# pain7576/ddpg-trucktrailer

Measured on AMD Instinct MI355X. Metric: env-steps/s, higher is better.
Workload: dtype f64

## Files before the change

ddpg-trucktrailer_amd/csrc/ttenv.hip:

```cpp
#include <hip/hip_runtime.h>
#include <hip/hip_ext.h>

#include <cmath>
#include <cstdarg>
#include <cstdio>
#include <cstdlib>
#include <cstring>
#include <new>
#include <type_traits>
#include <vector>

#include "ttenv.h"
#include "tthost.h"
#include "ttphilox.h"

namespace {

#include "ttenv_math.h"
#include "ttenv_state.h"
#include "ttenv_step.h"
#include "ttenv_pose.h"
#include "ttenv_log.h"
#include "ttenv_hold.h"

#ifdef TT_STAMPS
#include "ttstamps.h"
__device__ unsigned long long g_stepblk[1024][2];
__device__ TTLog g_log_step;
#endif
#define TT_STEP_HEAD()                                                                                                                  \
    if (cursor) {                       \
        obs += (size_t)cursor[1] * n * OBS;                                                                                             \
        reward += (size_t)cursor[0] * n;                                                                                                \
        done += (size_t)cursor[0] * n;                                                                                                  \
    }                                                                                                                                   \
    const int block_first = blockIdx.x * BLOCK;                                                                                         \
    const int i = block_first + threadIdx.x;                                                                                            \
    const bool valid = i < n;                                                                                                           \
    const int nv = min(BLOCK, n - block_first);                                                                                         \
    float of[OBS];                                                                                                                      \
                                                                                                                                        \
    if (b.counter && i == 0) *b.counter += 1
#define TT_STEP_LOADS()                                                                                                                 \
    Env e;                                                                                                                              \
    load_env<PER_ENV>(P, b, i, e);                                                                                                      \
    float a = 0.f;                                                                                                                      \
    if (!RANDOM_POLICY) a = action[i]
#define TT_STEP_ACT()                                                                                                                   \
    if (RANDOM_POLICY) {                                                                                                                \
        a = random_action(policy_seed, (uint32_t)i, pk_steps(e.pk), b.episodes[i]);                                                     \
        if (action_out) action_out[i] = a;                                                                                              \
    }
#define TT_STEP_OUT()                                                                                                                   \
    if (P.nt) {                                                                                                                         \
        __builtin_nontemporal_store((float)o.total, reward + i);                                                                        \
        __builtin_nontemporal_store((uint8_t)(o.done ? 1 : 0), done + i);                                                               \
    } else {                                                                                                                            \
        reward[i] = (float)o.total;                                                                                                     \
        done[i] = o.done ? 1 : 0;                                                                                                       \
    }                                                                                                                                   \
    if (INFO) write_info(info, (size_t)n, i, e, o)
#define TT_STEP_RESET()                                                                                                                 \
    if (AUTO_RESET && o.done) {                                                                                                         \
        const uint32_t ep = b.episodes[i] + 1u;                                                                                         \
        b.episodes[i] = ep;                                                                                                             \
        double sx, sy, syaw;                                                                                                            \
        random_pose(P, seed, (uint32_t)i, ep, sx, sy, syaw);                                                                            \
        const Goal g0{P.gx, P.gy, P.sg, P.cg};                                                                                          \
        place_env(P, b, i, e, sx, sy, syaw, g0, P.gyaw, e.L2, of);                                                                      \
    }                                                                                                                                   \
    store_env(b, i, e)
#define TT_STEP_RETURN()                                                                                                                \
    ret += o.total;                                                                                                                     \
    lg.acc[i] = o.done ? 0.0 : ret;                               \
    const uint32_t len = pk_steps(e.pk)
#define TT_STEP_LAUNCH_COUNT()                                                                                                          \
    if (threadIdx.x == 0) {                                                                                                             \
        const unsigned long long launch = __hip_atomic_load(lg.hdr + LG_LAUNCHES, __ATOMIC_RELAXED, __HIP_MEMORY_SCOPE_AGENT);          \
        const unsigned long long t = atomic_add_agent(lg.hdr + LG_TICKET, 1ull);                                                        \
        if (t == gridDim.x - 1u) {                               \
            __hip_atomic_store(lg.hdr + LG_TICKET, 0ull, __ATOMIC_RELAXED, __HIP_MEMORY_SCOPE_AGENT);                                   \
            __hip_atomic_store(lg.hdr + LG_LAUNCHES, launch + 1ull, __ATOMIC_RELAXED, __HIP_MEMORY_SCOPE_AGENT);                        \
        }                                                                                                                               \
    }

template <bool PER_ENV, bool INFO, bool AUTO_RESET, bool RANDOM_POLICY>
__global__ __launch_bounds__(BLOCK) void k_step(const KParams P, const int n, const Bufs b,
                                                const float *__restrict__ action, float *__restrict__ action_out,
                                                float *__restrict__ obs, float *__restrict__ reward,
                                                uint8_t *__restrict__ done, const Info info, const uint64_t seed,
                                                const uint64_t policy_seed, const int *__restrict__ cursor) {
    __shared__ __attribute__((aligned(16))) float tile[BLOCK * OBS];
#ifdef TT_STAMPS
    if (threadIdx.x == 0 && blockIdx.x < 1024) g_stepblk[blockIdx.x][0] = wall_clock64();
#endif
    TT_STEP_HEAD();
    if (valid) {
        TT_STEP_LOADS();
        __builtin_amdgcn_sched_barrier(0);
        TT_STEP_ACT();
        StepOut o;
#ifdef TT_DBG_STEP_MEM_ONLY
        o = StepOut{};
        o.total = e.psi1 + a; o.done = false;
        e.psi1 += 1e-9; e.psi2 += e.x1 * 1e-12; e.d3 = e.d2; e.d2 = e.d1; e.d1 = e.prev; e.cum += e.closest * 1e-12;
#pragma unroll
        for (int j = 0; j < OBS; ++j) of[j] = (float)(e.x2 + j);
#else
        step_env(P, e, a, of, o);
#endif
        TT_STEP_OUT();
        TT_STEP_RESET();
    }
    store_obs_tile(tile, of, valid, obs, block_first, nv, P.nt != 0);
#ifdef TT_STAMPS
    asm volatile("s_waitcnt vmcnt(0)" ::: "memory");
    __syncthreads();
    if (threadIdx.x == 0 && blockIdx.x < 1024) {
        g_stepblk[blockIdx.x][1] = wall_clock64();
        tt_log_add(g_log_step, g_stepblk[blockIdx.x][0], g_stepblk[blockIdx.x][1]);
    }
#endif
}

template <bool PER_ENV, bool INFO, bool AUTO_RESET, bool RANDOM_POLICY>
__global__ __launch_bounds__(BLOCK) void k_step_log(const KParams P, const int n, const Bufs b,
                                                    const float *__restrict__ action, float *__restrict__ action_out,
                                                    float *__restrict__ obs, float *__restrict__ reward,
                                                    uint8_t *__restrict__ done, const Info info, const uint64_t seed,
                                                    const uint64_t policy_seed, const int *__restrict__ cursor,
                                                    const EpLog lg) {
    __shared__ __attribute__((aligned(16))) float tile[BLOCK * OBS];
    TT_STEP_HEAD();
    if (valid) {
        TT_STEP_LOADS();
        double ret = lg.acc[i];
        __builtin_amdgcn_sched_barrier(0);
        TT_STEP_ACT();
        StepOut o;
        step_env(P, e, a, of, o);
        TT_STEP_OUT();
        TT_STEP_RETURN();
        TT_STEP_RESET();
        log_append(lg, i, o.done, o.flags, o.final_bonus > 0.0, len, ret);
    }
    store_obs_tile(tile, of, valid, obs, block_first, nv, P.nt != 0);
    TT_STEP_LAUNCH_COUNT();
}

template <bool PER_ENV, bool INFO, bool AUTO_RESET, bool RANDOM_POLICY>
__global__ __launch_bounds__(BLOCK) void k_step_tally(const KParams P, const int n, const Bufs b,
                                                      const float *__restrict__ action, float *__restrict__ action_out,
                                                      float *__restrict__ obs, float *__restrict__ reward,
                                                      uint8_t *__restrict__ done, const Info info, const uint64_t seed,
                                                      const uint64_t policy_seed, const int *__restrict__ cursor,
                                                      const EpLog lg) {
    __shared__ __attribute__((aligned(16))) float tile[BLOCK * OBS];
    TT_STEP_HEAD();
    if (valid) {
        TT_STEP_LOADS();
        double ret = lg.acc[i];
        __builtin_amdgcn_sched_barrier(0);
        TT_STEP_ACT();
        StepOut o;
        step_env(P, e, a, of, o);
        TT_STEP_OUT();
        TT_STEP_RETURN();
        double s0 = 0.0, s1 = 0.0, s2 = 0.0;
        if (o.done) {
            const double *cold = b.cold + i;
            const size_t S = (size_t)P.npad;
            s0 = cold[C_SX * S]; s1 = cold[C_SY * S]; s2 = cold[C_SYAW * S];
        }
        TT_STEP_RESET();
        tally_append(P, lg, i, o, len, ret, s0, s1, s2);
    }
    store_obs_tile(tile, of, valid, obs, block_first, nv, P.nt != 0);
    TT_STEP_LAUNCH_COUNT();
}

template <bool PER_ENV>
__global__ __launch_bounds__(BLOCK) void k_rollout(const KParams P, const int n, const Bufs b, const int k_steps,
                                                   float *__restrict__ obs, float *__restrict__ reward_sum,
                                                   int32_t *__restrict__ episodes_done, const uint64_t seed,
                                                   const uint64_t policy_seed) {
    __shared__ __attribute__((aligned(16))) float tile[BLOCK * OBS];
    const int block_first = blockIdx.x * BLOCK;
    const int i = block_first + threadIdx.x;
    const bool valid = i < n;
    float of[OBS];
    if (valid) {
        Env e;
        load_env<PER_ENV>(P, b, i, e);
        uint32_t ep = b.episodes[i];
        double rsum = 0.0;
        int ndone = 0;
        for (int t = 0; t < k_steps; ++t) {
            const float a = random_action(policy_seed, (uint32_t)i, pk_steps(e.pk), ep);
            StepOut o;
            step_env(P, e, a, of, o);
            rsum += o.total;
            if (o.done) {
                ep += 1u;
                ndone += 1;
                double sx, sy, syaw;
                random_pose(P, seed, (uint32_t)i, ep, sx, sy, syaw);
                const Goal g0{P.gx, P.gy, P.sg, P.cg};
                place_env(P, b, i, e, sx, sy, syaw, g0, P.gyaw, e.L2, of);
            }
        }
// ... 60 lines not shown
    va_end(ap);
    if (e) std::memcpy(e->err, g_err, tthost::ERR_BYTES);
    return code;
}

#define TT_HANDLE(env)                                                                       \
    do {                                                                                     \
        if (!(env)) return fail(nullptr, TT_EINVAL, "%s: NULL handle", __func__);            \
    } while (0)
#define TT_ENTER(env)                                                                        \
    do {                                                                                     \
        TT_HANDLE(env);                                                                      \
        TT_HIP(env, hipSetDevice(env->device));                                              \
    } while (0)

#define TT_HIP(e, call)                                                                      \
    do {                                                                                     \
        hipError_t err_ = (call);                                                            \
        if (err_ != hipSuccess) return fail((e), TT_EHIP, "%s: %s", #call, hipGetErrorString(err_)); \
    } while (0)

#define TT_LAUNCH(env, ...)                                                                  \
    do {                                                                                     \
        __VA_ARGS__;                                                                         \
        TT_HIP(env, hipGetLastError());                                                      \
    } while (0)
#define TT_RUN(env, ...)                                                                     \
    do {                                                                                     \
        TT_HIP(env, hipSetDevice(env->device));                                              \
        TT_LAUNCH(env, __VA_ARGS__);                                                         \
        return TT_OK;                                                                        \
    } while (0)

inline int nt_stores_for(int npad) {
    static const long long thr = [] {
        const char *e = std::getenv("TT_NT_ENVS");
        return e ? std::atoll(e) : 2097152ll;
    }();
    return thr > 0 && npad >= thr ? 1 : 0;
}

KParams make_kparams(const tt_params &p, int npad) {
    KParams k{};
    k.v = p.v1x;
    k.v_over_L1 = p.v1x / p.L1;
    k.ho = p.hitch_offset;
    k.h = p.dt;
    k.L2 = p.L2;
    k.gx = p.goal[0]; k.gy = p.goal[1]; k.gyaw = p.goal[2];
    k.sg = std::sin(p.goal[2]); k.cg = std::cos(p.goal[2]);
    k.minx = p.map_min_x; k.maxx = p.map_max_x; k.miny = p.map_min_y; k.maxy = p.map_max_y;
    const double w = p.map_max_x - p.map_min_x, hgt = p.map_max_y - p.map_min_y;
    k.cx = (p.map_max_x + p.map_min_x) / 2; k.cy = (p.map_max_y + p.map_min_y) / 2;
    k.inv_hx = 1.0 / (w / 2); k.inv_hy = 1.0 / (hgt / 2);
    k.inv_M = 1.0 / std::sqrt(w * w + hgt * hgt);
    k.max_steer = p.max_steer;
    k.pos_thr = p.position_threshold; k.ori_thr = p.orientation_threshold;
    k.step_length = p.step_length;
    k.inv_step_length = 1.0 / p.step_length;
    for (int i = 0; i < 3; ++i) { k.rlo[i] = p.reset_lo[i]; k.rhi[i] = p.reset_hi[i]; }
    k.extra_steps = p.extra_steps; k.fixed_max = p.fixed_max_steps;
    k.term_mask = p.term_mask;
    k.npad = npad;
    k.stateless = p.stateless_reward;
    k.pool_m = 0;
    k.pool = nullptr;
    k.nt = nt_stores_for(npad);
    return k;
}

inline int grid_for(int n) { return (n + BLOCK - 1) / BLOCK; }

// ... 5 lines not shown

template <bool PER_ENV, bool INFO, bool RANDOM_POLICY>
void launch_step(tt_env *e, bool auto_reset, const float *action, float *action_out, float *obs, float *reward,
                 uint8_t *done, const Info &info, uint64_t policy_seed, hipStream_t s, const int *cursor = nullptr) {
    const dim3 g(grid_for(e->n)), b(BLOCK);
    hipEvent_t t0 = nullptr, t1 = nullptr;
    if (e->profiling && e->ev_used < e->ev_start.size()) {
        t0 = e->ev_start[e->ev_used];
        t1 = e->ev_stop[e->ev_used];
        e->ev_used += 1;
    }
    const auto launch = [&](auto kernel, const auto &...log) {
        hipExtLaunchKernelGGL(kernel, g, b, 0, s, t0, t1, 0, e->kp, e->n, e->b, action, action_out, obs, reward, done, info, e->seed,
                              policy_seed, cursor, log...);
    };
    if (e->task_dev && auto_reset) {
        const TaskDev *tk = e->task_dev;
        if (e->log_bytes) launch(k_step_task_log<INFO, RANDOM_POLICY>, e->log, tk);
        else launch(k_step_task<INFO, RANDOM_POLICY>, tk);
    } else if (e->rnd_dev && auto_reset) {
        const RndDev *rnd = e->rnd_dev;
        if (e->log_bytes) launch(k_step_rnd_log<INFO, RANDOM_POLICY>, e->log, rnd);
        else launch(k_step_rnd<INFO, RANDOM_POLICY>, rnd);
    } else if (e->cur_dev && auto_reset) {
        const CurDev *cur = e->cur_dev;
        if (e->log_bytes) launch(k_step_cur_log<PER_ENV, INFO, RANDOM_POLICY>, e->log, cur);
        else launch(k_step_cur<PER_ENV, INFO, RANDOM_POLICY>, cur);
    } else if (e->log_flags & TT_LOG_DETAIL) {
        if (auto_reset) launch(k_step_tally<PER_ENV, INFO, true, RANDOM_POLICY>, e->log);
        else launch(k_step_tally<PER_ENV, INFO, false, RANDOM_POLICY>, e->log);
    } else if (e->log_bytes) {
        if (auto_reset) launch(k_step_log<PER_ENV, INFO, true, RANDOM_POLICY>, e->log);
        else launch(k_step_log<PER_ENV, INFO, false, RANDOM_POLICY>, e->log);
    } else if (auto_reset)
        launch(k_step<PER_ENV, INFO, true, RANDOM_POLICY>);
    else
        launch(k_step<PER_ENV, INFO, false, RANDOM_POLICY>);
}

template <bool RANDOM_POLICY>
int step_common(tt_env *env, const float *action, float *action_out, float *obs, float *reward, uint8_t *done,
                const tt_info *info, int auto_reset, uint64_t policy_seed, hipStream_t stream, const int *cursor = nullptr) {
    Info ki{nullptr, nullptr, nullptr};
    bool want_info = false;
    if (info) {
        ki.comp = info->comp; ki.violation = info->violation; ki.flags = info->flags;
        want_info = ki.comp || ki.violation || ki.flags;
    }
    const auto launch = [&](auto per_env, auto with_info) {
        launch_step<decltype(per_env)::value, decltype(with_info)::value, RANDOM_POLICY>(env, auto_reset != 0, action, action_out, obs,
                                                                                         reward, done, ki, policy_seed, stream, cursor);
    };
    by_per_env(env, [&](auto per_env) {
        if (want_info) launch(per_env, std::true_type{});
        else launch(per_env, std::false_type{});
    });
    hipError_t err = hipGetLastError();
    if (err != hipSuccess) return fail(env, TT_EHIP, "tt_env_step launch: %s", hipGetErrorString(err));
    return TT_OK;
}

constexpr long long kLogMaxCapacity = 1ll << 28;
inline int log_acc_rows(uint32_t flags) { return (flags & TT_LOG_DETAIL) ? 1 + TT_LOG_NCOMP : 1; }
size_t log_acc_offset(long long cap, uint32_t flags) {
    return log_records_bytes((unsigned long long)cap) + ((flags & TT_LOG_DETAIL) ? tally_records_bytes((unsigned long long)cap) : 0);
}
// ... 1003 lines not shown
```

ddpg-trucktrailer_amd/csrc/ttenv_curriculum.h:

```cpp
#pragma once

struct CurDev {
    uint32_t *cell;
    uint32_t *cum;
    uint32_t *attempts, *successes;
    int C, nx, ny, nyaw;
    uint32_t *q;
    double *p;
    unsigned long long *seen;
    int mode, reserved_;
    double alpha, uniform;
    double lo[3], width[3];
    unsigned long long seed;
};

__device__ __forceinline__ void curriculum_pose(const CurDev *cur, uint64_t seed, uint32_t env, uint32_t episode, double &sx,
                                                double &sy, double &syaw) {
#pragma clang fp contract(off)
    uint32_t r[4];
    philox4x32(env, episode, 0u, 0x7452u, (uint32_t)seed, (uint32_t)(seed >> 32), r);
    const uint32_t *cum = cur->cum;
    const int C = cur->C;
    const uint32_t t = (uint32_t)(((unsigned long long)r[3] * (unsigned long long)cum[C - 1]) >> 32);
    uint32_t lo = 0u;
// ... 29 lines not shown
        ncell = (uint32_t)cur->C;                                                                                                       \
    }                                                                                                                                   \
    if (cl < ncell) __hip_atomic_fetch_add(cur->attempts + cl, 1u, __ATOMIC_RELAXED, __HIP_MEMORY_SCOPE_AGENT);                         \
    if (cl < ncell && o.final_bonus > 0.0) __hip_atomic_fetch_add(cur->successes + cl, 1u, __ATOMIC_RELAXED, __HIP_MEMORY_SCOPE_AGENT); \
    if (o.done) {                                                                                                                       \
        const uint32_t ep = *ep_ptr + 1u;                                                                                               \
        *ep_ptr = ep;                                                                                                                   \
        double sx, sy, syaw;                                                                                                            \
        curriculum_pose(cur, cur->seed, (uint32_t)i, ep, sx, sy, syaw);                                                                 \
        const Goal g0{P.gx, P.gy, P.sg, P.cg};                                                                                          \
        place_env(P, b, i, e, sx, sy, syaw, g0, P.gyaw, e.L2, of);                                                                      \
    }                                                                                                                                   \
    store_env(b, i, e)

template <bool PER_ENV, bool INFO, bool RANDOM_POLICY>
__global__ __launch_bounds__(BLOCK) void k_step_cur(const KParams P, const int n, const Bufs b,
                                                    const float *__restrict__ action, float *__restrict__ action_out,
                                                    float *__restrict__ obs, float *__restrict__ reward,
                                                    uint8_t *__restrict__ done, const Info info, const uint64_t seed,
                                                    const uint64_t policy_seed, const int *__restrict__ cursor,
                                                    const CurDev *cur_arg) {
    __shared__ __attribute__((aligned(16))) float tile[BLOCK * OBS];
    TT_STEP_HEAD();
    TT_STEP_CUR();
    if (valid) {
        TT_STEP_LOADS();
        __builtin_amdgcn_sched_barrier(0);
        TT_STEP_ACT();
        StepOut o;
        step_env(P, e, a, of, o);
        TT_STEP_OUT();
        TT_STEP_RESET_CURRICULUM();
    }
    store_obs_tile(tile, of, valid, obs, block_first, nv, P.nt != 0);
}

template <bool PER_ENV, bool INFO, bool RANDOM_POLICY>
__global__ __launch_bounds__(BLOCK) void k_step_cur_log(const KParams P, const int n, const Bufs b,
                                                        const float *__restrict__ action, float *__restrict__ action_out,
                                                        float *__restrict__ obs, float *__restrict__ reward,
                                                        uint8_t *__restrict__ done, const Info info, const uint64_t seed,
                                                        const uint64_t policy_seed, const int *__restrict__ cursor,
                                                        const EpLog lg, const CurDev *cur_arg) {
    __shared__ __attribute__((aligned(16))) float tile[BLOCK * OBS];
    TT_STEP_HEAD();
    TT_STEP_CUR();
    if (valid) {
        TT_STEP_LOADS();
        double ret = lg.acc[i];
        __builtin_amdgcn_sched_barrier(0);
        TT_STEP_ACT();
        StepOut o;
        step_env(P, e, a, of, o);
        TT_STEP_OUT();
        TT_STEP_RETURN();
        TT_STEP_RESET_CURRICULUM();
        log_append(lg, i, o.done, o.flags, o.final_bonus > 0.0, len, ret);
    }
    store_obs_tile(tile, of, valid, obs, block_first, nv, P.nt != 0);
    TT_STEP_LAUNCH_COUNT();
}

__global__ __launch_bounds__(BLOCK) void k_reset_curriculum(const KParams P, const int n, const Bufs b, const uint8_t *mask,
                                                            float *obs, const uint64_t seed, const CurDev *cur) {
    reset_lane(P, n, b, mask, obs, [&](uint32_t env, uint32_t episode, double &sx, double &sy, double &syaw) {
        curriculum_pose(cur, seed, env, episode, sx, sy, syaw);
    });
}

__global__ void k_curriculum_seed(CurDev *cur, const uint64_t seed) { cur->seed = seed; }

__global__ __launch_bounds__(BLOCK) void k_curriculum_unset(const int n, const int k, const int32_t *idx, uint32_t *cell) {
    const int j = blockIdx.x * BLOCK + threadIdx.x;
    int i;
    if (!lane_of_entry(idx, k, n, j, i)) return;
    cell[i] = TT_CURRICULUM_NO_CELL;
}

__global__ __launch_bounds__(BLOCK) void k_curriculum_update(const CurDev *cur) {
#pragma clang fp contract(off)
    __shared__ uint32_t part[BLOCK];
    const int C = cur->C, tid = threadIdx.x;
    const int per = (C + BLOCK - 1) / BLOCK;
    const int first = min(C, tid * per), last = min(C, first + per);
    const double alpha = cur->alpha, u = cur->uniform;
    const bool hard = cur->mode == TT_CURRICULUM_HARD;
    uint32_t sum = 0u;
    for (int c = first; c < last; ++c) {
        double p = cur->p[c];
        const uint32_t na = cur->attempts[c];
        if (na > 0u) {
            const uint32_t s = cur->successes[c];
// ... 28 lines not shown
```

ddpg-trucktrailer_amd/csrc/ttenv_hold.h:

```cpp
#pragma once

struct HoldCols {
    double *ret, *end;
    int32_t *len;
    uint8_t *live, *flags, *success;
};
__host__ __device__ inline size_t hold_block_bytes(int npad) { return (4 * sizeof(double) + sizeof(int32_t) + 3) * (size_t)npad; }
__host__ __device__ inline HoldCols hold_cols(void *block, int npad) {
    const size_t S = (size_t)npad;
    HoldCols c;
    c.ret = static_cast<double *>(block);
    c.end = c.ret + S;
    c.len = reinterpret_cast<int32_t *>(c.end + 3 * S);
    c.live = reinterpret_cast<uint8_t *>(c.len + S);
    c.flags = c.live + S;
    c.success = c.flags + S;
    return c;
}

__device__ inline void load_obs_tile(float *tile, const float *obs, int block_first, int nv) {
    const int tid = threadIdx.x;
    const float *src = obs + (size_t)block_first * OBS;
    const int total = nv * OBS;
    if ((reinterpret_cast<uintptr_t>(src) & 15u) == 0) {
// ... 10 lines not shown

template <bool PER_ENV>
__global__ __launch_bounds__(BLOCK) void k_step_hold(const KParams P, const int n, const Bufs b, const float *__restrict__ mu,
                                                     const float action_scale, float *__restrict__ obs, void *const hold) {
    __shared__ __attribute__((aligned(16))) float tile[BLOCK * OBS];
    const int block_first = blockIdx.x * BLOCK;
    const int i = block_first + threadIdx.x;
    const int nv = min(BLOCK, n - block_first);
    const HoldCols h = hold_cols(hold, P.npad);
    const bool live = i < n && h.live[i] != 0;
    const int nlive = __syncthreads_count(live ? 1 : 0);
    if (nlive == 0) return;
    if (nlive < nv) load_obs_tile(tile, obs, block_first, nv);
    float of[OBS];
    if (live) {
        Env e;
        load_env<PER_ENV>(P, b, i, e);
        float a = mu[i];
        __builtin_amdgcn_sched_barrier(0);
        a = a * action_scale;
        StepOut o;
        step_env(P, e, a, of, o);
        h.ret[i] += o.total;
        store_env(b, i, e);
        if (o.done) {
            const size_t S = (size_t)P.npad;
            h.len[i] = (int32_t)pk_steps(e.pk);
            h.flags[i] = (uint8_t)o.flags;
            h.success[i] = o.final_bonus > 0.0 ? 1 : 0;
            h.end[i] = e.x2; h.end[S + i] = e.y2; h.end[2 * S + i] = e.psi2;
            h.live[i] = 0;
        }
    }
    store_obs_tile(tile, of, live, obs, block_first, nv, P.nt != 0);
}

__global__ __launch_bounds__(BLOCK) void k_hold_begin(const int n, const int npad, void *const hold) {
    const int i = blockIdx.x * BLOCK + threadIdx.x;
    if (i >= npad) return;
    const HoldCols h = hold_cols(hold, npad);
    const size_t S = (size_t)npad;
    h.live[i] = i < n ? 1 : 0;
    h.ret[i] = 0.0;
    h.len[i] = 0;
    h.flags[i] = 0;
    h.success[i] = 0;
    h.end[i] = 0.0; h.end[S + i] = 0.0; h.end[2 * S + i] = 0.0;
}

__global__ __launch_bounds__(BLOCK) void k_hold_live(const int npad, const void *const hold, long long *out) {
    __shared__ long long part[BLOCK];
    const uint32_t *w = reinterpret_cast<const uint32_t *>(hold_cols(const_cast<void *>(hold), npad).live);
    long long s = 0;
    for (int q = threadIdx.x; q < (npad >> 2); q += BLOCK) {
        const uint32_t x = w[q];
        s += (long long)((x & 0xFFu) + ((x >> 8) & 0xFFu) + ((x >> 16) & 0xFFu) + (x >> 24));
    }
    part[threadIdx.x] = s;
    __syncthreads();
    for (int d = BLOCK >> 1; d > 0; d >>= 1) {
        if ((int)threadIdx.x < d) part[threadIdx.x] += part[threadIdx.x + d];
        __syncthreads();
    }
    if (threadIdx.x == 0) *out = part[0];
}

__global__ __launch_bounds__(BLOCK) void k_hold_read(const int n, const int npad, void *const hold, double *ret, int32_t *len,
// ... 12 lines not shown
```

ddpg-trucktrailer_amd/csrc/ttenv_randomize.h:

```cpp
#pragma once

struct RndDev {
    double glo[3], gw[3];
    double l2lo, l2w;
    unsigned long long seed;
    double rlo[3], rhi[3];
    const double *pool;
    int pool_m, reserved_;
};

__device__ __forceinline__ void randomized_task(const RndDev *rnd, uint64_t seed, uint32_t env, uint32_t episode, Goal &g, double &gyaw,
                                                double &L2) {
#pragma clang fp contract(off)
    uint32_t r[4];
    philox4x32(env, episode, 1u, 0x7452u, (uint32_t)seed, (uint32_t)(seed >> 32), r);
    g.gx = rnd->glo[0] + rnd->gw[0] * u01(r[0]);
    g.gy = rnd->glo[1] + rnd->gw[1] * u01(r[1]);
    gyaw = rnd->glo[2] + rnd->gw[2] * u01(r[2]);
    L2 = rnd->l2lo + rnd->l2w * u01(r[3]);
    tt_sincos(kTable, gyaw, g.sg, g.cg);
}

__device__ __forceinline__ void randomized_start(const RndDev *rnd, uint64_t seed, uint32_t env, uint32_t episode, double &sx,
                                                 double &sy, double &syaw) {
// ... 17 lines not shown
#define TT_STEP_RESET_RANDOMIZED()                                                                                                      \
    if (o.done) {                                                                                                                       \
        const uint32_t ep = *ep_ptr + 1u;                                                                                               \
        *ep_ptr = ep;                                                                                                                   \
        const uint64_t rseed = rnd->seed;                                                                                               \
        double sx, sy, syaw, gyaw, l2;                                                                                                  \
        randomized_start(rnd, rseed, (uint32_t)i, ep, sx, sy, syaw);                                                                    \
        Goal g1;                                                                                                                        \
        randomized_task(rnd, rseed, (uint32_t)i, ep, g1, gyaw, l2);                                                                     \
        place_env(P, b, i, e, sx, sy, syaw, g1, gyaw, l2, of);                                                                          \
    }                                                                                                                                   \
    store_env(b, i, e)

template <bool INFO, bool RANDOM_POLICY>
__global__ __launch_bounds__(BLOCK) void k_step_rnd(const KParams P, const int n, const Bufs b,
                                                    const float *__restrict__ action, float *__restrict__ action_out,
                                                    float *__restrict__ obs, float *__restrict__ reward,
                                                    uint8_t *__restrict__ done, const Info info, const uint64_t seed,
                                                    const uint64_t policy_seed, const int *__restrict__ cursor,
                                                    const RndDev *rnd_arg) {
    constexpr bool PER_ENV = true;
    __shared__ __attribute__((aligned(16))) float tile[BLOCK * OBS];
    TT_STEP_HEAD();
    TT_STEP_RND();
    if (valid) {
        TT_STEP_LOADS();
        __builtin_amdgcn_sched_barrier(0);
        TT_STEP_ACT();
        StepOut o;
        step_env(P, e, a, of, o);
        TT_STEP_OUT();
        TT_STEP_RESET_RANDOMIZED();
    }
    store_obs_tile(tile, of, valid, obs, block_first, nv, P.nt != 0);
}

template <bool INFO, bool RANDOM_POLICY>
__global__ __launch_bounds__(BLOCK) void k_step_rnd_log(const KParams P, const int n, const Bufs b,
                                                        const float *__restrict__ action, float *__restrict__ action_out,
                                                        float *__restrict__ obs, float *__restrict__ reward,
                                                        uint8_t *__restrict__ done, const Info info, const uint64_t seed,
                                                        const uint64_t policy_seed, const int *__restrict__ cursor,
                                                        const EpLog lg, const RndDev *rnd_arg) {
    constexpr bool PER_ENV = true;
    __shared__ __attribute__((aligned(16))) float tile[BLOCK * OBS];
    TT_STEP_HEAD();
    TT_STEP_RND();
    if (valid) {
        TT_STEP_LOADS();
        double ret = lg.acc[i];
        __builtin_amdgcn_sched_barrier(0);
        TT_STEP_ACT();
        StepOut o;
        step_env(P, e, a, of, o);
        TT_STEP_OUT();
        TT_STEP_RETURN();
        TT_STEP_RESET_RANDOMIZED();
        log_append(lg, i, o.done, o.flags, o.final_bonus > 0.0, len, ret);
    }
    store_obs_tile(tile, of, valid, obs, block_first, nv, P.nt != 0);
    TT_STEP_LAUNCH_COUNT();
}

__global__ __launch_bounds__(BLOCK) void k_reset_rnd(const KParams P, const int n, const Bufs b, const uint8_t *mask, float *obs,
                                                     const uint64_t seed, const RndDev *rnd) {
    reset_lane(
        P, n, b, mask, obs,
        [&](uint32_t env, uint32_t episode, double &sx, double &sy, double &syaw) { random_pose(P, seed, env, episode, sx, sy, syaw); },
        [&](uint32_t env, uint32_t episode, Goal &g, double &gyaw, double &L2) { randomized_task(rnd, seed, env, episode, g, gyaw, L2); });
}

__global__ void k_rnd_seed(RndDev *rnd, const uint64_t seed) { rnd->seed = seed; }
```

ddpg-trucktrailer_amd/csrc/ttenv_state.h:

```cpp
#pragma once

constexpr int OBS = TT_OBS_DIM;
#ifndef TT_BLOCK
#define TT_BLOCK 256
#endif
constexpr int BLOCK = TT_BLOCK;
constexpr int TILE = 64;

enum HotRow : int {
    H_PSI1 = 0, H_PSI2, H_X1, H_Y1, H_X2, H_Y2,
    H_D3, H_D2, H_D1, H_PREV, H_CUM, H_CLOSEST,
    H_DINIT,
    H_MISC,
    H_ROWS
};
enum ColdRow : int { C_SX = 0, C_SY, C_SYAW, C_GX, C_GY, C_GYAW, C_SG, C_CG, C_L2, C_ROWS };

__host__ __device__ inline uint32_t pk_steps(uint32_t p) { return p & 0xFFFu; }
__host__ __device__ inline uint32_t pk_max(uint32_t p) { return (p >> 12) & 0xFFFu; }
__host__ __device__ inline uint32_t pk_stages(uint32_t p) { return (p >> 24) & 0x3u; }
__host__ __device__ inline uint32_t pk_age(uint32_t p) { return p >> 26; }
__host__ __device__ inline uint32_t pk_make(uint32_t steps, uint32_t maxs, uint32_t stages, uint32_t age) {
    return (steps > 0xFFFu ? 0xFFFu : steps) | ((maxs > 0xFFFu ? 0xFFFu : maxs) << 12) | ((stages & 3u) << 24) |
           ((age > 63u ? 63u : age) << 26);
// ... 30 lines not shown
    return hot + (size_t)(i >> 6) * (H_ROWS * TILE) + (i & (TILE - 1));
}

__device__ __forceinline__ bool lane_of_entry(const int32_t *idx, int k, int n, int j, int &i) {
    if (j >= k) return false;
    i = idx ? idx[j] : j;
    return i >= 0 && i < n;
}

struct Goal {
    double gx, gy, sg, cg;
};

__device__ __forceinline__ void observe(const KParams &P, const Goal &g, double x1, double y1, double x2, double y2,
                                        double s1, double c1, double s2, double c2, double sd, double cd, double dx,
                                        double dy, double cur, double inv_cur, float *of) {
    const double dxl = dx * c2 + dy * s2, dyl = -dx * s2 + dy * c2;
    of[0] = (float)((x1 - P.cx) * P.inv_hx); of[1] = (float)((y1 - P.cy) * P.inv_hy);
    of[2] = (float)s1; of[3] = (float)c1;
    of[4] = (float)((x2 - P.cx) * P.inv_hx); of[5] = (float)((y2 - P.cy) * P.inv_hy);
    of[6] = (float)s2; of[7] = (float)c2;
    of[8] = (float)(s1 * c2 - c1 * s2); of[9] = (float)(c1 * c2 + s1 * s2);
    of[10] = (float)sd; of[11] = (float)cd;
    of[12] = (float)((g.gx - P.cx) * P.inv_hx); of[13] = (float)((g.gy - P.cy) * P.inv_hy);
    of[14] = (float)g.sg; of[15] = (float)g.cg;
    of[16] = (float)fmin(fmax(cur * P.inv_M, 0.0), 1.0);
    of[17] = (float)fmin(fmax(dxl * P.inv_M, -1.0), 1.0);
    of[18] = (float)fmin(fmax(dyl * P.inv_M, -1.0), 1.0);
    of[19] = (float)(g.sg * c2 - g.cg * s2); of[20] = (float)(g.cg * c2 + g.sg * s2);
    of[21] = (float)(cur > 0.0 ? -dyl * inv_cur : s2);
    of[22] = (float)(cur > 0.0 ? -dxl * inv_cur : -c2);
}

__device__ inline void store_obs_tile(float *tile, const float *of, bool valid, float *obs, int block_first, int nv,
                                      const bool nt = false) {
    const int tid = threadIdx.x;
    if (valid) {
#pragma unroll
        for (int j = 0; j < OBS; ++j) tile[tid * OBS + j] = of[j];
    }
    __syncthreads();
    float *dst = obs + (size_t)block_first * OBS;
    const int total = nv * OBS;
    if ((reinterpret_cast<uintptr_t>(dst) & 15u) == 0) {
        const int nvec = total >> 2;
        const float4 *t4 = reinterpret_cast<const float4 *>(tile);
        float4 *d4 = reinterpret_cast<float4 *>(dst);
        if (nt) {
            using v4f = __attribute__((ext_vector_type(4))) float;
            for (int q = tid; q < nvec; q += BLOCK) {
                const float4 t = t4[q];
                __builtin_nontemporal_store(v4f{t.x, t.y, t.z, t.w}, reinterpret_cast<v4f *>(d4 + q));
            }
        } else {
            for (int q = tid; q < nvec; q += BLOCK) d4[q] = t4[q];
        }
        for (int q = (nvec << 2) + tid; q < total; q += BLOCK) dst[q] = tile[q];
    } else {
        for (int q = tid; q < total; q += BLOCK) dst[q] = tile[q];
    }
    __syncthreads();
}

struct Env {
    double psi1, psi2, x1, y1, x2, y2;
    double d3, d2, d1, prev, cum, closest;
    double dinit;
    float psteer;
    uint32_t pk;
    Goal g;
    double gyaw, L2;
};

template <bool PER_ENV>
__device__ __forceinline__ void load_env(const KParams &P, const Bufs &b, int i, Env &e) {
    const double *h = hot_ptr(b.hot, i);
    e.psi1 = h[H_PSI1 * TILE]; e.psi2 = h[H_PSI2 * TILE];
    e.x1 = h[H_X1 * TILE]; e.y1 = h[H_Y1 * TILE]; e.x2 = h[H_X2 * TILE]; e.y2 = h[H_Y2 * TILE];
    e.d3 = h[H_D3 * TILE]; e.d2 = h[H_D2 * TILE]; e.d1 = h[H_D1 * TILE]; e.prev = h[H_PREV * TILE];
    e.cum = h[H_CUM * TILE]; e.closest = h[H_CLOSEST * TILE];
    e.dinit = h[H_DINIT * TILE];
    const uint2 m = *reinterpret_cast<const uint2 *>(h + H_MISC * TILE);
    e.psteer = __uint_as_float(m.x);
    e.pk = m.y;
    if (PER_ENV) {
        const double *c = b.cold + i;
        const size_t S = (size_t)P.npad;
        e.g.gx = c[C_GX * S]; e.g.gy = c[C_GY * S]; e.g.sg = c[C_SG * S]; e.g.cg = c[C_CG * S];
        e.gyaw = c[C_GYAW * S]; e.L2 = c[C_L2 * S];
    } else {
        e.g.gx = P.gx; e.g.gy = P.gy; e.g.sg = P.sg; e.g.cg = P.cg;
        e.gyaw = P.gyaw; e.L2 = P.L2;
    }
}

__device__ __forceinline__ void store_env(const Bufs &b, int i, const Env &e) {
    double *h = hot_ptr(b.hot, i);
    h[H_PSI1 * TILE] = e.psi1; h[H_PSI2 * TILE] = e.psi2;
    h[H_X1 * TILE] = e.x1; h[H_Y1 * TILE] = e.y1; h[H_X2 * TILE] = e.x2; h[H_Y2 * TILE] = e.y2;
    h[H_D3 * TILE] = e.d3; h[H_D2 * TILE] = e.d2; h[H_D1 * TILE] = e.d1; h[H_PREV * TILE] = e.prev;
    h[H_CUM * TILE] = e.cum; h[H_CLOSEST * TILE] = e.closest;
    *reinterpret_cast<uint2 *>(h + H_MISC * TILE) = make_uint2(__float_as_uint(e.psteer), e.pk);
}

__device__ inline void place_env(const KParams &P, const Bufs &b, int i, Env &e, double sx, double sy, double syaw,
                                 const Goal &g, double gyaw, double L2, float *of) {
    const KTable &T = kTable;
    double ss, cs;
    tt_sincos(T, syaw, ss, cs);
    e.psi1 = e.psi2 = (double)(float)syaw;
    e.x1 = (double)(float)(sx + L2 * cs);
    e.y1 = (double)(float)(sy + L2 * ss);
    e.x2 = (double)(float)sx;
    e.y2 = (double)(float)sy;
    const double ddx = g.gx - sx, ddy = g.gy - sy;
    e.dinit = sqrt(ddx * ddx + ddy * ddy);
    e.g = g; e.gyaw = gyaw; e.L2 = L2;
    const int maxs = P.fixed_max > 0 ? P.fixed_max : (int)(e.dinit / P.step_length) + P.extra_steps;
    e.pk = pk_make(0u, (uint32_t)maxs, 0u, 0u);
    e.d3 = e.d2 = e.d1 = e.prev = e.closest = e.dinit; e.cum = 0.0; e.psteer = 0.0f;
    hot_ptr(b.hot, i)[H_DINIT * TILE] = e.dinit;
    double *c = b.cold + i;
    const size_t S = (size_t)P.npad;
    c[C_SX * S] = sx; c[C_SY * S] = sy; c[C_SYAW * S] = syaw;
    c[C_GX * S] = g.gx; c[C_GY * S] = g.gy; c[C_GYAW * S] = gyaw; c[C_SG * S] = g.sg; c[C_CG * S] = g.cg;
    c[C_L2 * S] = L2;
    if (of) {
        double sp, cp;
        tt_sincos(T, e.psi1, sp, cp);
        const double dx = g.gx - e.x2, dy = g.gy - e.y2;
        const double cur = sqrt(dx * dx + dy * dy);
        observe(P, g, e.x1, e.y1, e.x2, e.y2, sp, cp, sp, cp, 0.0, 1.0, dx, dy, cur, cur > 0.0 ? 1.0 / cur : 0.0, of);
    }
}

// ... 20 lines not shown
```

ddpg-trucktrailer_amd/csrc/ttenv_task.h:

```cpp
#pragma once

struct TaskDev {
    CurDev cur;
    RndDev rnd;
    double cw[4];
    int bins[4];
};
static_assert(offsetof(TaskDev, cur) == 0, "k_curriculum_update takes the descriptor's address as a CurDev's");

__device__ __forceinline__ void task_draw(const TaskDev *tk, uint64_t seed, uint32_t env, uint32_t episode, Goal &g, double &gyaw,
                                          double &L2) {
#pragma clang fp contract(off)
    uint32_t r[4], s[4];
    philox4x32(env, episode, 1u, 0x7452u, (uint32_t)seed, (uint32_t)(seed >> 32), r);
    philox4x32(env, episode, 2u, 0x7452u, (uint32_t)seed, (uint32_t)(seed >> 32), s);
    const uint32_t *cum = tk->cur.cum;
    const int C = tk->cur.C;
    const uint32_t t = (uint32_t)(((unsigned long long)s[0] * (unsigned long long)cum[C - 1]) >> 32);
    uint32_t lo = 0u;
#pragma unroll
    for (uint32_t h = TT_CURRICULUM_MAX_CELLS / 2; h > 0u; h >>= 1) {
        const uint32_t j = lo + h;
        const uint32_t v = cum[min(j, (uint32_t)C) - 1u];
        lo = (j <= (uint32_t)C && v <= t) ? j : lo;
// ... 28 lines not shown
        __hip_atomic_fetch_add(tk->cur.successes + cl, 1u, __ATOMIC_RELAXED, __HIP_MEMORY_SCOPE_AGENT);                                 \
    if (o.done) {                                                                                                                       \
        const uint32_t ep = *ep_ptr + 1u;                                                                                               \
        *ep_ptr = ep;                                                                                                                   \
        const uint64_t rseed = tk->rnd.seed;                                                                                            \
        double sx, sy, syaw, gyaw, l2;                                                                                                  \
        randomized_start(&tk->rnd, rseed, (uint32_t)i, ep, sx, sy, syaw);                                                               \
        Goal g1;                                                                                                                        \
        task_draw(tk, rseed, (uint32_t)i, ep, g1, gyaw, l2);                                                                            \
        place_env(P, b, i, e, sx, sy, syaw, g1, gyaw, l2, of);                                                                          \
    }                                                                                                                                   \
    store_env(b, i, e)

template <bool INFO, bool RANDOM_POLICY>
__global__ __launch_bounds__(BLOCK) void k_step_task(const KParams P, const int n, const Bufs b,
                                                     const float *__restrict__ action, float *__restrict__ action_out,
                                                     float *__restrict__ obs, float *__restrict__ reward,
                                                     uint8_t *__restrict__ done, const Info info, const uint64_t seed,
                                                     const uint64_t policy_seed, const int *__restrict__ cursor,
                                                     const TaskDev *tk_arg) {
    constexpr bool PER_ENV = true;
    __shared__ __attribute__((aligned(16))) float tile[BLOCK * OBS];
    TT_STEP_HEAD();
    TT_STEP_TASK();
    if (valid) {
        TT_STEP_LOADS();
        __builtin_amdgcn_sched_barrier(0);
        TT_STEP_ACT();
        StepOut o;
        step_env(P, e, a, of, o);
        TT_STEP_OUT();
        TT_STEP_RESET_TASK();
    }
    store_obs_tile(tile, of, valid, obs, block_first, nv, P.nt != 0);
}

template <bool INFO, bool RANDOM_POLICY>
__global__ __launch_bounds__(BLOCK) void k_step_task_log(const KParams P, const int n, const Bufs b,
                                                         const float *__restrict__ action, float *__restrict__ action_out,
                                                         float *__restrict__ obs, float *__restrict__ reward,
                                                         uint8_t *__restrict__ done, const Info info, const uint64_t seed,
                                                         const uint64_t policy_seed, const int *__restrict__ cursor,
                                                         const EpLog lg, const TaskDev *tk_arg) {
    constexpr bool PER_ENV = true;
    __shared__ __attribute__((aligned(16))) float tile[BLOCK * OBS];
    TT_STEP_HEAD();
    TT_STEP_TASK();
    if (valid) {
        TT_STEP_LOADS();
        double ret = lg.acc[i];
        __builtin_amdgcn_sched_barrier(0);
        TT_STEP_ACT();
        StepOut o;
        step_env(P, e, a, of, o);
        TT_STEP_OUT();
        TT_STEP_RETURN();
        TT_STEP_RESET_TASK();
        log_append(lg, i, o.done, o.flags, o.final_bonus > 0.0, len, ret);
    }
    store_obs_tile(tile, of, valid, obs, block_first, nv, P.nt != 0);
    TT_STEP_LAUNCH_COUNT();
}

__global__ __launch_bounds__(BLOCK) void k_reset_task(const KParams P, const int n, const Bufs b, const uint8_t *mask, float *obs,
                                                      const uint64_t seed, const TaskDev *tk) {
    reset_lane(
        P, n, b, mask, obs,
        [&](uint32_t env, uint32_t episode, double &sx, double &sy, double &syaw) { random_pose(P, seed, env, episode, sx, sy, syaw); },
        [&](uint32_t env, uint32_t episode, Goal &g, double &gyaw, double &L2) { task_draw(tk, seed, env, episode, g, gyaw, L2); });
}
```

Before: 808.4 million.

## Add write-through store path for step kernel outputs and env state

Adds a k_step_wt kernel variant, chosen by default once the padded env count reaches 32768 and stays below the nontemporal threshold. It writes obs, reward, done and the hot env state with 16-byte global stores carrying the sc1 cache bit. Reward and done are staged per wave in LDS so they can go out as full vectors, and env-state pairs are exchanged between neighbouring lanes with DPP so each store is 16 bytes. The aim is fewer, wider store transactions and a changed cache policy for data the next step reads back. In exchange it uses inline asm with an extra s_nop, an explicit LDS wait, and falls back to plain stores for partial waves or misaligned buffers.

```diff
diff --git a/ddpg-trucktrailer_amd/csrc/ttenv.hip b/ddpg-trucktrailer_amd/csrc/ttenv.hip
--- a/ddpg-trucktrailer_amd/csrc/ttenv.hip
+++ b/ddpg-trucktrailer_amd/csrc/ttenv.hip
@@ -52,7 +52,7 @@
         if (action_out) action_out[i] = a;                                                                                              \
     }
 #define TT_STEP_OUT()                                                                                                                   \
-    if (P.nt) {                                                                                                                         \
+    if (P.nt == SF_NT) {                                                                                                                \
         __builtin_nontemporal_store((float)o.total, reward + i);                                                                        \
         __builtin_nontemporal_store((uint8_t)(o.done ? 1 : 0), done + i);                                                               \
     } else {                                                                                                                            \
@@ -60,7 +60,7 @@
         done[i] = o.done ? 1 : 0;                                                                                                       \
     }                                                                                                                                   \
     if (INFO) write_info(info, (size_t)n, i, e, o)
-#define TT_STEP_RESET()                                                                                                                 \
+#define TT_STEP_PLACE()                                                                                                                 \
     if (AUTO_RESET && o.done) {                                                                                                         \
         const uint32_t ep = b.episodes[i] + 1u;                                                                                         \
         b.episodes[i] = ep;                                                                                                             \
@@ -68,8 +68,25 @@
         random_pose(P, seed, (uint32_t)i, ep, sx, sy, syaw);                                                                            \
         const Goal g0{P.gx, P.gy, P.sg, P.cg};                                                                                          \
         place_env(P, b, i, e, sx, sy, syaw, g0, P.gyaw, e.L2, of);                                                                      \
-    }                                                                                                                                   \
+    }
+#define TT_STEP_RESET()                                                                                                                 \
+    TT_STEP_PLACE();                                                                                                                    \
     store_env(b, i, e)
+#define TT_WT_WAVE(form) (P.nt >= (form) && (__builtin_amdgcn_readfirstlane(i) | 63) < n)
+#define TT_WT_SLOT(arr) (TT_WT_WAVE(SF_WT) && (reinterpret_cast<uintptr_t>(arr) & 15u) == 0)
+#define TT_STEP_OUT_WT()                                                                                                                \
+    rew_f = (float)o.total;                             \
+    done_b = o.done ? 1u : 0u;                                                                                                          \
+    if (!TT_WT_SLOT(reward)) reward[i] = rew_f;                                                                                         \
+    if (!TT_WT_SLOT(done)) done[i] = (uint8_t)done_b;                                                                                   \
+    if (INFO) write_info(info, (size_t)n, i, e, o)
+#define TT_STEP_RESET_WT()                                                                                                              \
+    TT_STEP_PLACE();                                                                                                                    \
+    if (TT_WT_WAVE(SF_WT_HOT)) store_env_wt(b, i, e);                                                                                   \
+    else store_env(b, i, e)
+#define TT_STEP_TILE_WT()                                                                                                               \
+    store_obs_tile(tile, of, valid, obs, block_first, nv, P.nt);                                                                        \
+    store_rd_tile(tile, TT_WT_SLOT(reward), TT_WT_SLOT(done), rew_f, done_b, reward, done, i)
 #define TT_STEP_RETURN()                                                                                                                \
     ret += o.total;                                                                                                                     \
     lg.acc[i] = o.done ? 0.0 : ret;                               \
@@ -112,7 +129,48 @@
         TT_STEP_OUT();
         TT_STEP_RESET();
     }
-    store_obs_tile(tile, of, valid, obs, block_first, nv, P.nt != 0);
+    store_obs_tile(tile, of, valid, obs, block_first, nv, P.nt == SF_NT);
+#ifdef TT_STAMPS
+    asm volatile("s_waitcnt vmcnt(0)" ::: "memory");
+    __syncthreads();
+    if (threadIdx.x == 0 && blockIdx.x < 1024) {
+        g_stepblk[blockIdx.x][1] = wall_clock64();
+        tt_log_add(g_log_step, g_stepblk[blockIdx.x][0], g_stepblk[blockIdx.x][1]);
+    }
+#endif
+}
+
+template <bool PER_ENV, bool INFO, bool AUTO_RESET, bool RANDOM_POLICY>
+__global__ __launch_bounds__(BLOCK) void k_step_wt(const KParams P, const int n, const Bufs b,
+                                                const float *__restrict__ action, float *__restrict__ action_out,
+                                                float *__restrict__ obs, float *__restrict__ reward,
+                                                uint8_t *__restrict__ done, const Info info, const uint64_t seed,
+                                                const uint64_t policy_seed, const int *__restrict__ cursor) {
+    __shared__ __attribute__((aligned(16))) float tile[BLOCK * OBS];
+#ifdef TT_STAMPS
+    if (threadIdx.x == 0 && blockIdx.x < 1024) g_stepblk[blockIdx.x][0] = wall_clock64();
+#endif
+    TT_STEP_HEAD();
+    float rew_f = 0.f;
+    uint32_t done_b = 0u;
+    if (valid) {
+        TT_STEP_LOADS();
+        __builtin_amdgcn_sched_barrier(0);
+        TT_STEP_ACT();
+        StepOut o;
+#ifdef TT_DBG_STEP_MEM_ONLY
+        o = StepOut{};
+        o.total = e.psi1 + a; o.done = false;
+        e.psi1 += 1e-9; e.psi2 += e.x1 * 1e-12; e.d3 = e.d2; e.d2 = e.d1; e.d1 = e.prev; e.cum += e.closest * 1e-12;
+#pragma unroll
+        for (int j = 0; j < OBS; ++j) of[j] = (float)(e.x2 + j);
+#else
+        step_env(P, e, a, of, o);
+#endif
+        TT_STEP_OUT_WT();
+        TT_STEP_RESET_WT();
+    }
+    TT_STEP_TILE_WT();
 #ifdef TT_STAMPS
     asm volatile("s_waitcnt vmcnt(0)" ::: "memory");
     __syncthreads();
@@ -144,7 +202,7 @@
         TT_STEP_RESET();
         log_append(lg, i, o.done, o.flags, o.final_bonus > 0.0, len, ret);
     }
-    store_obs_tile(tile, of, valid, obs, block_first, nv, P.nt != 0);
+    store_obs_tile(tile, of, valid, obs, block_first, nv, P.nt == SF_NT);
     TT_STEP_LAUNCH_COUNT();
 }
 
@@ -175,7 +233,7 @@
         TT_STEP_RESET();
         tally_append(P, lg, i, o, len, ret, s0, s1, s2);
     }
-    store_obs_tile(tile, of, valid, obs, block_first, nv, P.nt != 0);
+    store_obs_tile(tile, of, valid, obs, block_first, nv, P.nt == SF_NT);
     TT_STEP_LAUNCH_COUNT();
 }
 
@@ -302,12 +360,16 @@
         return TT_OK;                                                                        \
     } while (0)
 
+constexpr int kWtMinEnvs = 32768;
 inline int nt_stores_for(int npad) {
-    static const long long thr = [] {
-        const char *e = std::getenv("TT_NT_ENVS");
-        return e ? std::atoll(e) : 2097152ll;
-    }();
-    return thr > 0 && npad >= thr ? 1 : 0;
+    long long thr = 2097152ll;
+    int below = npad >= kWtMinEnvs ? SF_WT_HOT : SF_PLAIN;
+    if (const char *e = std::getenv("TT_NT_ENVS")) {
+        if (!std::strcmp(e, "wt")) below = SF_WT;
+        else if (!std::strcmp(e, "wt-hot")) below = SF_WT_HOT;
+        else { thr = std::atoll(e); below = SF_PLAIN; }
+    }
+    return thr > 0 && npad >= thr ? SF_NT : below;
 }
 
 KParams make_kparams(const tt_params &p, int npad) {
@@ -379,6 +441,9 @@
     } else if (e->log_bytes) {
         if (auto_reset) launch(k_step_log<PER_ENV, INFO, true, RANDOM_POLICY>, e->log);
         else launch(k_step_log<PER_ENV, INFO, false, RANDOM_POLICY>, e->log);
+    } else if (e->kp.nt >= SF_WT) {
+        if (auto_reset) launch(k_step_wt<PER_ENV, INFO, true, RANDOM_POLICY>);
+        else launch(k_step_wt<PER_ENV, INFO, false, RANDOM_POLICY>);
     } else if (auto_reset)
         launch(k_step<PER_ENV, INFO, true, RANDOM_POLICY>);
     else
diff --git a/ddpg-trucktrailer_amd/csrc/ttenv_curriculum.h b/ddpg-trucktrailer_amd/csrc/ttenv_curriculum.h
--- a/ddpg-trucktrailer_amd/csrc/ttenv_curriculum.h
+++ b/ddpg-trucktrailer_amd/csrc/ttenv_curriculum.h
@@ -85,7 +85,7 @@
         TT_STEP_OUT();
         TT_STEP_RESET_CURRICULUM();
     }
-    store_obs_tile(tile, of, valid, obs, block_first, nv, P.nt != 0);
+    store_obs_tile(tile, of, valid, obs, block_first, nv, P.nt == SF_NT);
 }
 
 template <bool PER_ENV, bool INFO, bool RANDOM_POLICY>
@@ -110,7 +110,7 @@
         TT_STEP_RESET_CURRICULUM();
         log_append(lg, i, o.done, o.flags, o.final_bonus > 0.0, len, ret);
     }
-    store_obs_tile(tile, of, valid, obs, block_first, nv, P.nt != 0);
+    store_obs_tile(tile, of, valid, obs, block_first, nv, P.nt == SF_NT);
     TT_STEP_LAUNCH_COUNT();
 }
 
diff --git a/ddpg-trucktrailer_amd/csrc/ttenv_hold.h b/ddpg-trucktrailer_amd/csrc/ttenv_hold.h
--- a/ddpg-trucktrailer_amd/csrc/ttenv_hold.h
+++ b/ddpg-trucktrailer_amd/csrc/ttenv_hold.h
@@ -66,7 +66,7 @@
             h.live[i] = 0;
         }
     }
-    store_obs_tile(tile, of, live, obs, block_first, nv, P.nt != 0);
+    store_obs_tile(tile, of, live, obs, block_first, nv, P.nt == SF_NT);
 }
 
 __global__ __launch_bounds__(BLOCK) void k_hold_begin(const int n, const int npad, void *const hold) {
diff --git a/ddpg-trucktrailer_amd/csrc/ttenv_randomize.h b/ddpg-trucktrailer_amd/csrc/ttenv_randomize.h
--- a/ddpg-trucktrailer_amd/csrc/ttenv_randomize.h
+++ b/ddpg-trucktrailer_amd/csrc/ttenv_randomize.h
@@ -73,7 +73,7 @@
         TT_STEP_OUT();
         TT_STEP_RESET_RANDOMIZED();
     }
-    store_obs_tile(tile, of, valid, obs, block_first, nv, P.nt != 0);
+    store_obs_tile(tile, of, valid, obs, block_first, nv, P.nt == SF_NT);
 }
 
 template <bool INFO, bool RANDOM_POLICY>
@@ -99,7 +99,7 @@
         TT_STEP_RESET_RANDOMIZED();
         log_append(lg, i, o.done, o.flags, o.final_bonus > 0.0, len, ret);
     }
-    store_obs_tile(tile, of, valid, obs, block_first, nv, P.nt != 0);
+    store_obs_tile(tile, of, valid, obs, block_first, nv, P.nt == SF_NT);
     TT_STEP_LAUNCH_COUNT();
 }
 
diff --git a/ddpg-trucktrailer_amd/csrc/ttenv_state.h b/ddpg-trucktrailer_amd/csrc/ttenv_state.h
--- a/ddpg-trucktrailer_amd/csrc/ttenv_state.h
+++ b/ddpg-trucktrailer_amd/csrc/ttenv_state.h
@@ -86,8 +86,15 @@
     of[22] = (float)(cur > 0.0 ? -dxl * inv_cur : -c2);
 }
 
+enum StoreForm : int { SF_PLAIN = 0, SF_NT = 1, SF_WT = 2, SF_WT_HOT = 3 };
+
+using u32x4 = __attribute__((ext_vector_type(4))) unsigned;
+__device__ __forceinline__ void st_wt16(void *p, const u32x4 v) {
+    asm volatile("global_store_dwordx4 %0, %1, off sc1\n\ts_nop 1" : : "v"(p), "v"(v) : "memory");
+}
+
 __device__ inline void store_obs_tile(float *tile, const float *of, bool valid, float *obs, int block_first, int nv,
-                                      const bool nt = false) {
+                                      const int form = SF_PLAIN) {
     const int tid = threadIdx.x;
     if (valid) {
 #pragma unroll
@@ -100,11 +107,16 @@
         const int nvec = total >> 2;
         const float4 *t4 = reinterpret_cast<const float4 *>(tile);
         float4 *d4 = reinterpret_cast<float4 *>(dst);
-        if (nt) {
+        if (form == SF_NT) {
             using v4f = __attribute__((ext_vector_type(4))) float;
             for (int q = tid; q < nvec; q += BLOCK) {
                 const float4 t = t4[q];
                 __builtin_nontemporal_store(v4f{t.x, t.y, t.z, t.w}, reinterpret_cast<v4f *>(d4 + q));
+            }
+        } else if (form >= SF_WT) {
+            for (int q = tid; q < nvec; q += BLOCK) {
+                const float4 t = t4[q];
+                st_wt16(d4 + q, u32x4{__float_as_uint(t.x), __float_as_uint(t.y), __float_as_uint(t.z), __float_as_uint(t.w)});
             }
         } else {
             for (int q = tid; q < nvec; q += BLOCK) d4[q] = t4[q];
@@ -155,6 +167,42 @@
     h[H_D3 * TILE] = e.d3; h[H_D2 * TILE] = e.d2; h[H_D1 * TILE] = e.d1; h[H_PREV * TILE] = e.prev;
     h[H_CUM * TILE] = e.cum; h[H_CLOSEST * TILE] = e.closest;
     *reinterpret_cast<uint2 *>(h + H_MISC * TILE) = make_uint2(__float_as_uint(e.psteer), e.pk);
+}
+
+__device__ __forceinline__ uint32_t pair_swap(const uint32_t v) {
+    return (uint32_t)__builtin_amdgcn_update_dpp(0, (int)v, 0xB1, 0xf, 0xf, true);
+}
+__device__ __forceinline__ double pair_swap(const double v) {
+    const uint64_t u = __builtin_bit_cast(uint64_t, v);
+    return __builtin_bit_cast(double, ((uint64_t)pair_swap((uint32_t)(u >> 32)) << 32) | (uint64_t)pair_swap((uint32_t)u));
+}
+
+__device__ __forceinline__ void store_env_wt(const Bufs &b, int i, const Env &e) {
+    const bool odd = (i & 1) != 0;
+    double *const h = hot_ptr(b.hot, i & ~1);
+    const auto rows2 = [&](const int ra, const double va, const double vb) __attribute__((always_inline)) {
+        const double got = pair_swap(odd ? va : vb);
+        const uint64_t lo = __builtin_bit_cast(uint64_t, odd ? got : va), hi = __builtin_bit_cast(uint64_t, odd ? vb : got);
+        st_wt16(h + (ra + (odd ? 1 : 0)) * TILE, u32x4{(unsigned)lo, (unsigned)(lo >> 32), (unsigned)hi, (unsigned)(hi >> 32)});
+    };
+    rows2(H_PSI1, e.psi1, e.psi2); rows2(H_X1, e.x1, e.y1); rows2(H_X2, e.x2, e.y2);
+    rows2(H_D3, e.d3, e.d2); rows2(H_D1, e.d1, e.prev); rows2(H_CUM, e.cum, e.closest);
+    const uint32_t m0 = __float_as_uint(e.psteer), n0 = pair_swap(m0), n1 = pair_swap(e.pk);
+    if (!odd) st_wt16(h + H_MISC * TILE, u32x4{m0, e.pk, n0, n1});
+}
+
+__device__ __forceinline__ void store_rd_tile(float *tile, const bool rew_v, const bool done_v, const float rew, const uint32_t dn,
+                                              float *reward, uint8_t *done, const int i) {
+    if (!(rew_v || done_v)) return;
+    const int lane = threadIdx.x & 63, w0 = threadIdx.x & ~63;
+    const int first = i & ~63;
+    float *const tr = tile + w0;
+    uint8_t *const td = reinterpret_cast<uint8_t *>(tile + BLOCK) + w0;
+    tr[lane] = rew;
+    td[lane] = (uint8_t)dn;
+    asm volatile("s_waitcnt lgkmcnt(0)" ::: "memory");
+    if (rew_v && lane < 16) st_wt16(reward + first + 4 * lane, reinterpret_cast<const u32x4 *>(tr)[lane]);
+    if (done_v && lane >= 16 && lane < 20) st_wt16(done + first + 16 * (lane - 16), reinterpret_cast<const u32x4 *>(td)[lane - 16]);
 }
 
 __device__ inline void place_env(const KParams &P, const Bufs &b, int i, Env &e, double sx, double sy, double syaw,
diff --git a/ddpg-trucktrailer_amd/csrc/ttenv_task.h b/ddpg-trucktrailer_amd/csrc/ttenv_task.h
--- a/ddpg-trucktrailer_amd/csrc/ttenv_task.h
+++ b/ddpg-trucktrailer_amd/csrc/ttenv_task.h
@@ -84,7 +84,7 @@
         TT_STEP_OUT();
         TT_STEP_RESET_TASK();
     }
-    store_obs_tile(tile, of, valid, obs, block_first, nv, P.nt != 0);
+    store_obs_tile(tile, of, valid, obs, block_first, nv, P.nt == SF_NT);
 }
 
 template <bool INFO, bool RANDOM_POLICY>
@@ -110,7 +110,7 @@
         TT_STEP_RESET_TASK();
         log_append(lg, i, o.done, o.flags, o.final_bonus > 0.0, len, ret);
     }
-    store_obs_tile(tile, of, valid, obs, block_first, nv, P.nt != 0);
+    store_obs_tile(tile, of, valid, obs, block_first, nv, P.nt == SF_NT);
     TT_STEP_LAUNCH_COUNT();
 }
 
```

After: 791.6 million. -2.1%, worse.
